# mj129/Tramba

Measured on AMD Instinct MI355X. Metric: images/sec fwd Tramba-V 384x384, higher is better.
Workload: dtype bf16; 1 GPU; Tramba-V (VMamba-B encoder) 384x384 bf16 inference, batch 4 per GPU, random-init weights (seed 1026), randn images; global_batch=4, launch=hipGraph replay, decoder guide branches on a side stream

## Files before the change

### tramba_amd/csrc/linear.hip

```cpp
#include <stdlib.h>
#include <string.h>

#include <type_traits>

#include "common.h"

namespace tramba {

typedef __attribute__((ext_vector_type(8))) short frag8_t;
typedef __attribute__((ext_vector_type(8))) _Float16 frag8h_t;
typedef __attribute__((ext_vector_type(16))) float acc16_t;

template <typename T> struct Mfma;
template <> struct Mfma<__hip_bfloat16> {
    static constexpr int KSTEP = 16;
    using frag = frag8_t;
    static __device__ __forceinline__ acc16_t run(frag a, frag b, acc16_t c)
    {
        typedef __attribute__((ext_vector_type(8))) __bf16 bf8;
        return __builtin_amdgcn_mfma_f32_32x32x16_bf16(__builtin_bit_cast(bf8, a), __builtin_bit_cast(bf8, b), c, 0, 0, 0);
    }
};
template <> struct Mfma<__half> {
    static constexpr int KSTEP = 16;
// ... 694 lines not shown
    TRAMBA_DSR128_(a[3], aa[3], S); TRAMBA_DSR128_(b[3], ba[3], S)
        if constexpr ((STG & 3) == 0) { TRAMBA_RD_STG_(0, 4096); }
        else if constexpr ((STG & 3) == 1) { TRAMBA_RD_STG_(16384, 20480); }
        else if constexpr ((STG & 3) == 2) { TRAMBA_RD_STG_(32768, 36864); }
        else { TRAMBA_RD_STG_(49152, 53248); }
#undef TRAMBA_RD_STG_
        if constexpr (LNIN) {
            asm volatile("s_waitcnt lgkmcnt(8)" : "+v"(sv[0]), "+v"(sv[1]) : : "memory");
#pragma unroll
            for (int i = 0; i < 2; ++i)
#pragma unroll
                for (int e = 0; e < 4; ++e) {
                    rs1[i] = dot2_ones<T>(sv[i][e], rs1[i]);
                    rs2[i] = dot2_self<T>(sv[i][e], rs2[i]);
                }
        }
        asm volatile("s_waitcnt lgkmcnt(6)" : "+v"(a[0]), "+v"(b[0]) : : "memory");
        acc[0][0] = Mfma<T>::run(b[0], a[0], acc[0][0]);
        asm volatile("s_waitcnt lgkmcnt(4)" : "+v"(a[1]), "+v"(b[1]) : : "memory");
        acc[0][0] = Mfma<T>::run(b[1], a[1], acc[0][0]);
        asm volatile("s_waitcnt lgkmcnt(2)" : "+v"(a[2]), "+v"(b[2]) : : "memory");
        acc[0][0] = Mfma<T>::run(b[2], a[2], acc[0][0]);
        asm volatile("s_waitcnt lgkmcnt(0)" : "+v"(a[3]), "+v"(b[3]) : : "memory");
        acc[0][0] = Mfma<T>::run(b[3], a[3], acc[0][0]);
    };
    int kt0 = 0;
    for (; kt0 + NSTG <= nk; kt0 += NSTG) {
        kstep(kt0, std::integral_constant<int, 0>{});
        kstep(kt0 + 1, std::integral_constant<int, 1>{});
        if constexpr (NSTG > 2) kstep(kt0 + 2, std::integral_constant<int, 2>{});
        if constexpr (NSTG > 3) kstep(kt0 + 3, std::integral_constant<int, 3>{});
        if constexpr (NSTG > 4) {
            kstep(kt0 + 4, std::integral_constant<int, 4>{});
            kstep(kt0 + 5, std::integral_constant<int, 5>{});
            kstep(kt0 + 6, std::integral_constant<int, 6>{});
            kstep(kt0 + 7, std::integral_constant<int, 7>{});
        }
    }
    if (kt0 < nk) kstep(kt0, std::integral_constant<int, 0>{});
    if constexpr (NSTG > 2) {
        if (kt0 + 1 < nk) kstep(kt0 + 1, std::integral_constant<int, 1>{});
    }
    if constexpr (NSTG > 3) {
        if (kt0 + 2 < nk) kstep(kt0 + 2, std::integral_constant<int, 2>{});
    }
    if constexpr (NSTG > 4) {
        if (kt0 + 3 < nk) kstep(kt0 + 3, std::integral_constant<int, 3>{});
        if (kt0 + 4 < nk) kstep(kt0 + 4, std::integral_constant<int, 4>{});
        if (kt0 + 5 < nk) kstep(kt0 + 5, std::integral_constant<int, 5>{});
        if (kt0 + 6 < nk) kstep(kt0 + 6, std::integral_constant<int, 6>{});
    }
    __syncthreads();
    if constexpr (LNIN) {
        float2 *rowstat = reinterpret_cast<float2 *>(lds + LDS_BYTES);
#pragma unroll
        for (int i = 0; i < 2; ++i) {
            float s1 = rs1[i], s2 = rs2[i];
#pragma unroll
            for (int m = 1; m < 8; m <<= 1) {
                s1 += __shfl_xor(s1, m, 64);
                s2 += __shfl_xor(s2, m, 64);
            }
            const float mean = s1 / (float)K;
            const float var = fmaxf(s2 / (float)K - mean * mean, 0.f);
            if ((tid & 7) == 0) rowstat[(tid >> 3) + 32 * i] = make_float2(mean, rsqrtf(var + li.eps));
        }
        tile_epilogue<T, TO, BM, BN>(acc, lds, bias, res, y, M, N, act, m0, n0, li.colsum,
                                     reinterpret_cast<const float2 *>(lds + LDS_BYTES));
    } else {
        tile_epilogue<T, TO, BM, BN>(acc, lds, bias, res, y, M, N, act, m0, n0, nullptr, nullptr, DUAL ? y_pre : nullptr);
    }
#endif
}

enum { A_PLAIN = 0, A_TWO = 1, A_CONV = 2 };
struct ASrc {
    const void *x2;
    int k1;
    ConvGeom cg;
    unsigned abytes;
};

#define TRAMBA_DSR128_(OUT, ADDR, OFF) asm volatile("ds_read_b128 %0, %1 offset:" #OFF : "=v"(OUT) : "v"(ADDR) : "memory")
template <typename T, typename TO, int NSTG, bool LNIN = false, bool DUAL = false, int ASRC = A_PLAIN>
__global__ __launch_bounds__(512, ASRC == A_CONV && NSTG == 3 ? 6 : 1) void linear_pc_kernel(const T *__restrict__ x, const T *__restrict__ w,
                                                       const float *__restrict__ bias, const T *__restrict__ res,
                                                       TO *__restrict__ y, long M, int N, int K, int act,
                                                       LnIn li = LnIn{nullptr, 0.f}, TO *__restrict__ y_pre = nullptr,
                                                       ASrc as = ASrc{nullptr, 0, ConvGeom{0, 0, 0, 0, 0}, 0u})
{
#if defined(__HIP_DEVICE_COMPILE__)
    constexpr int BM = 64, BN = 64;
    constexpr int TILE_BYTES = (BM + BN) * kBK * 2;
    constexpr int EPI_BYTES = BM * (BN + 4) * 4;
    constexpr int LDS_BYTES = NSTG * TILE_BYTES > EPI_BYTES ? NSTG * TILE_BYTES : EPI_BYTES;
    static_assert(NSTG == 3 || NSTG == 4, "stage index = kt % NSTG with the loop unrolled by NSTG");
    __shared__ __attribute__((aligned(1024))) unsigned char lds[LDS_BYTES + (LNIN ? BM * 8 : 0)];
    typedef __attribute__((address_space(3))) void lds_void;

    const int tid = threadIdx.x, lane = tid & 63;
    const int wave = __builtin_amdgcn_readfirstlane(tid >> 6);
    const bool loader = wave >= 4;
    const int cw = wave & 3;
    const int wm = cw >> 1, wn = cw & 1;
    const int r32 = lane & 31, hi = lane >> 5;
    long m0;
    int n0;
    {
        const unsigned nblk = gridDim.x * gridDim.y, lin = blockIdx.y * gridDim.x + blockIdx.x;
        const unsigned q = nblk >> 3, r = nblk & 7, xcd = lin & 7, slot = lin >> 3;
        const unsigned t = xcd * q + (xcd < r ? xcd : r) + slot;
        m0 = (long)(t / gridDim.x) * BM;
        n0 = (int)(t % gridDim.x) * BN;
    }
    const int nk = K / kBK;
    const unsigned rowb = (unsigned)K * 2u;
    const long mrows = M - m0 < BM ? M - m0 : BM;
    const int nrows = N - n0 < BN ? N - n0 : BN;
    const bool stage_b = cw >= 2;
    __amdgpu_buffer_rsrc_t rs, rsx;
    unsigned voff[4];
    unsigned lx[4] = {0u, 0u, 0u, 0u}, ly[4] = {0u, 0u, 0u, 0u};
    unsigned(&voff2)[4] = lx;
    unsigned(&chy)[4] = lx, (&cwx)[4] = ly;
    int nsw = nk;
    unsigned hlim = 0xffffffffu, wlim = 0xffffffffu;
    int ccs = 0, cdy = 0, cdx = 0;
    if constexpr (ASRC == A_TWO) {
        const int ka = as.k1;
        const unsigned rowa = (unsigned)ka * 2u, rowa2 = (unsigned)(K - ka) * 2u;
        rs = stage_b ? make_rsrc(w + (long)n0 * K, (unsigned)nrows * rowb) : make_rsrc(x + m0 * ka, (unsigned)mrows * rowa);
        rsx = stage_b ? rs : make_rsrc((const T *)as.x2 + m0 * (K - ka), (unsigned)mrows * rowa2);
        if (!stage_b) nsw = ka / kBK;
#pragma unroll
        for (int j = 0; j < 4; ++j) {
            const int row = ((cw & 1) * 4 + j) * 8 + (lane >> 3);
            const int c = (lane & 7) ^ ((row >> 1) & 7);
            voff[j] = (unsigned)row * (stage_b ? rowb : rowa) + (unsigned)c * 16u;
            voff2[j] = (unsigned)row * (stage_b ? rowb : rowa2) + (unsigned)c * 16u;
        }
    } else if constexpr (ASRC == A_CONV) {
        rs = stage_b ? make_rsrc(w + (long)n0 * K, (unsigned)nrows * rowb) : make_rsrc(x, as.abytes);
        if (!stage_b) {
            hlim = (unsigned)as.cg.hin;
            wlim = (unsigned)as.cg.win;
        }
#pragma unroll
        for (int j = 0; j < 4; ++j) {
            const int row = ((cw & 1) * 4 + j) * 8 + (lane >> 3);
            const int c = (lane & 7) ^ ((row >> 1) & 7);
            if (stage_b) {
                voff[j] = (unsigned)row * rowb + (unsigned)c * 16u;
                chy[j] = cwx[j] = 0u;
            } else {
                const long gr = m0 + row;
                const bool ok = gr < M;
                const unsigned pix = ok ? (unsigned)gr : 0u;
                const unsigned wo = pix % (unsigned)as.cg.wout, t = pix / (unsigned)as.cg.wout;
                const unsigned ho = t % (unsigned)as.cg.hout, b = t / (unsigned)as.cg.hout;
                chy[j] = (unsigned)(ok ? 2 * (int)ho - 1 : -4);
                cwx[j] = (unsigned)(2 * (int)wo - 1);
                voff[j] = ((b * (unsigned)as.cg.hin + chy[j]) * (unsigned)as.cg.win + cwx[j]) * ((unsigned)as.cg.cin * 2u) +
                          (unsigned)c * 16u;
            }
        }
    } else {
        rs = stage_b ? make_rsrc(w + (long)n0 * K, (unsigned)nrows * rowb) : make_rsrc(x + m0 * K, (unsigned)mrows * rowb);
#pragma unroll
        for (int j = 0; j < 4; ++j) {
            const int row = ((cw & 1) * 4 + j) * 8 + (lane >> 3);
            const int c = (lane & 7) ^ ((row >> 1) & 7);
            voff[j] = (unsigned)row * rowb + (unsigned)c * 16u;
        }
    }
    unsigned char *mine = lds + (stage_b ? BM * kBK * 2 : 0) + (cw & 1) * 4096;
    auto issue = [&](int kt, int stg) {
        if constexpr (ASRC == A_TWO) {
            const bool first = kt < nsw;
            const __amdgpu_buffer_rsrc_t rsel = first ? rs : rsx;
            const unsigned so = (unsigned)(first ? kt : kt - nsw) * (kBK * 2);
#pragma unroll
            for (int j = 0; j < 4; ++j)
                __builtin_amdgcn_raw_ptr_buffer_load_lds(rsel, (lds_void *)(mine + stg * TILE_BYTES + j * 1024), 16,
                                                         first ? voff[j] : voff2[j], so, 0, 0);
        } else if constexpr (ASRC == A_CONV) {
            const unsigned so = stage_b ? (unsigned)kt * (kBK * 2)
                                        : (unsigned)((cdy * as.cg.win + cdx) * as.cg.cin + ccs * kBK) * 2u;
#pragma unroll
            for (int j = 0; j < 4; ++j) {
                const unsigned hy = chy[j] + (unsigned)cdy, wx = cwx[j] + (unsigned)cdx;
                unsigned out = (hy < hlim && wx < wlim) ? 0u : 1u;
                asm volatile("" : "+v"(out));
                __builtin_amdgcn_raw_ptr_buffer_load_lds(rs, (lds_void *)(mine + stg * TILE_BYTES + j * 1024), 16,
                                                         (voff[j] + so) | (out << 31), 0, 0, 0);
            }
            if (++ccs == as.cg.cin / kBK) {
                ccs = 0;
                if (++cdx == 3) { cdx = 0; ++cdy; }
            }
        } else {
            const unsigned so = (unsigned)kt * (kBK * 2);
#pragma unroll
            for (int j = 0; j < 4; ++j)
                __builtin_amdgcn_raw_ptr_buffer_load_lds(rs, (lds_void *)(mine + stg * TILE_BYTES + j * 1024), 16, voff[j], so,
                                                         0, 0);
        }
    };
    const unsigned lbase = (unsigned)(size_t)(__attribute__((address_space(3))) unsigned char *)lds;
    unsigned(&aad)[4] = lx, (&bad)[4] = ly;
    if (ASRC == A_PLAIN || !loader) {
        const int ra_ = wm * 32 + r32, rb_ = wn * 32 + r32;
        const unsigned a0 = lbase + (unsigned)(ra_ * 128 + ((hi ^ ((ra_ >> 1) & 7)) * 16));
        const unsigned b0 = lbase + (unsigned)(BM * kBK * 2 + rb_ * 128 + ((hi ^ ((rb_ >> 1) & 7)) * 16));
#pragma unroll
        for (int kk = 0; kk < 4; ++kk) {
            aad[kk] = a0 ^ (unsigned)(kk * 32);
            bad[kk] = b0 ^ (unsigned)(kk * 32);
        }
    }
    acc16_t acc[1][1];
#pragma unroll
    for (int r = 0; r < 16; ++r) acc[0][0][r] = 0.f;
    const int lt = tid & 255;
    float rs1[2] = {0.f, 0.f}, rs2[2] = {0.f, 0.f};
    const unsigned sad = lbase + (unsigned)((lt >> 3) * 128 + (lt & 7) * 16);

    constexpr int DEPTH = NSTG - 1;
    if (loader) {
#pragma unroll
        for (int t = 0; t < DEPTH; ++t)
            if (t < nk) issue(t, t);
    }
    auto kstep = [&](int kt, auto stg_c) {
        constexpr int STG = decltype(stg_c)::value;
        if (loader) {
            const int later = nk - 1 - kt;
            if (later >= DEPTH - 1) {
                if constexpr (DEPTH == 2) asm volatile("s_waitcnt vmcnt(4)" ::: "memory");
                else asm volatile("s_waitcnt vmcnt(8)" ::: "memory");
            } else {
                switch (later) {
                case 0: asm volatile("s_waitcnt vmcnt(0)" ::: "memory"); break;
                default: asm volatile("s_waitcnt vmcnt(4)" ::: "memory"); break;
                }
            }
        }
        __builtin_amdgcn_s_barrier();
        asm volatile("" ::: "memory");
        if (loader) {
            if (kt + DEPTH < nk) issue(kt + DEPTH, (STG + DEPTH) % NSTG);
        } else {
            frag8_t a[4], b[4];
            v4u_t sv[2];
            if constexpr (LNIN) {
                if constexpr (STG == 0) { TRAMBA_DSR128_(sv[0], sad, 0); TRAMBA_DSR128_(sv[1], sad, 4096); }
                else if constexpr (STG == 1) { TRAMBA_DSR128_(sv[0], sad, 16384); TRAMBA_DSR128_(sv[1], sad, 20480); }
                else if constexpr (STG == 2) { TRAMBA_DSR128_(sv[0], sad, 32768); TRAMBA_DSR128_(sv[1], sad, 36864); }
                else { TRAMBA_DSR128_(sv[0], sad, 49152); TRAMBA_DSR128_(sv[1], sad, 53248); }
            }
#define TRAMBA_RD_STG_(S)                                                                            \
    TRAMBA_DSR128_(a[0], aad[0], S); TRAMBA_DSR128_(b[0], bad[0], S); TRAMBA_DSR128_(a[1], aad[1], S); \
    TRAMBA_DSR128_(b[1], bad[1], S); TRAMBA_DSR128_(a[2], aad[2], S); TRAMBA_DSR128_(b[2], bad[2], S); \
    TRAMBA_DSR128_(a[3], aad[3], S); TRAMBA_DSR128_(b[3], bad[3], S)
            if constexpr (STG == 0) { TRAMBA_RD_STG_(0); }
            else if constexpr (STG == 1) { TRAMBA_RD_STG_(16384); }
            else if constexpr (STG == 2) { TRAMBA_RD_STG_(32768); }
            else { TRAMBA_RD_STG_(49152); }
#undef TRAMBA_RD_STG_
            if constexpr (LNIN) {
                asm volatile("s_waitcnt lgkmcnt(8)" : "+v"(sv[0]), "+v"(sv[1]) : : "memory");
#pragma unroll
                for (int i = 0; i < 2; ++i)
#pragma unroll
                    for (int e = 0; e < 4; ++e) {
                        rs1[i] = dot2_ones<T>(sv[i][e], rs1[i]);
                        rs2[i] = dot2_self<T>(sv[i][e], rs2[i]);
                    }
            }
            asm volatile("s_waitcnt lgkmcnt(6)" : "+v"(a[0]), "+v"(b[0]) : : "memory");
            acc[0][0] = Mfma<T>::run(b[0], a[0], acc[0][0]);
            __builtin_amdgcn_sched_barrier(0);
            asm volatile("s_waitcnt lgkmcnt(4)" : "+v"(a[1]), "+v"(b[1]) : : "memory");
            acc[0][0] = Mfma<T>::run(b[1], a[1], acc[0][0]);
            __builtin_amdgcn_sched_barrier(0);
            asm volatile("s_waitcnt lgkmcnt(2)" : "+v"(a[2]), "+v"(b[2]) : : "memory");
            acc[0][0] = Mfma<T>::run(b[2], a[2], acc[0][0]);
            __builtin_amdgcn_sched_barrier(0);
            asm volatile("s_waitcnt lgkmcnt(0)" : "+v"(a[3]), "+v"(b[3]) : : "memory");
            acc[0][0] = Mfma<T>::run(b[3], a[3], acc[0][0]);
        }
    };
    int kt0 = 0;
    for (; kt0 + NSTG <= nk; kt0 += NSTG) {
        kstep(kt0, std::integral_constant<int, 0>{});
        kstep(kt0 + 1, std::integral_constant<int, 1>{});
        kstep(kt0 + 2, std::integral_constant<int, 2>{});
        if constexpr (NSTG > 3) kstep(kt0 + 3, std::integral_constant<int, 3>{});
    }
    if (kt0 < nk) kstep(kt0, std::integral_constant<int, 0>{});
    if (kt0 + 1 < nk) kstep(kt0 + 1, std::integral_constant<int, 1>{});
    if constexpr (NSTG > 3) {
        if (kt0 + 2 < nk) kstep(kt0 + 2, std::integral_constant<int, 2>{});
    }
    __syncthreads();
    if constexpr (LNIN) {
        float2 *rowstat = reinterpret_cast<float2 *>(lds + LDS_BYTES);
        if (!loader) {
#pragma unroll
            for (int i = 0; i < 2; ++i) {
                float s1 = rs1[i], s2 = rs2[i];
#pragma unroll
                for (int m = 1; m < 8; m <<= 1) {
                    s1 += __shfl_xor(s1, m, 64);
                    s2 += __shfl_xor(s2, m, 64);
                }
                const float mean = s1 / (float)K;
                const float var = fmaxf(s2 / (float)K - mean * mean, 0.f);
                if ((lt & 7) == 0) rowstat[(lt >> 3) + 32 * i] = make_float2(mean, rsqrtf(var + li.eps));
            }
        }
        tile_epilogue<T, TO, BM, BN, 512>(acc, lds, bias, res, y, M, N, act, m0, n0, li.colsum,
                                          reinterpret_cast<const float2 *>(lds + LDS_BYTES));
    } else {
        tile_epilogue<T, TO, BM, BN, 512>(acc, lds, bias, res, y, M, N, act, m0, n0, nullptr, nullptr, DUAL ? y_pre : nullptr);
    }
#endif
}
#undef TRAMBA_DSR128_

template <typename T> __device__ __forceinline__ unsigned pack2_(float a, float b);
template <> __device__ __forceinline__ unsigned pack2_<__hip_bfloat16>(float a, float b)
{
    unsigned pk = 0u;
#if defined(__HIP_DEVICE_COMPILE__)
    asm("v_cvt_pk_bf16_f32 %0, %1, %2" : "=v"(pk) : "v"(a), "v"(b));
#endif
    return pk;
}
template <> __device__ __forceinline__ unsigned pack2_<__half>(float a, float b)
{
    unsigned pk = 0u;
#if defined(__HIP_DEVICE_COMPILE__)
    asm("v_cvt_pk_f16_f32 %0, %1, %2" : "=v"(pk) : "v"(a), "v"(b));
#endif
    return pk;
}
template <typename T> __device__ __forceinline__ float unpack_lo_(unsigned v);
template <typename T> __device__ __forceinline__ float unpack_hi_(unsigned v);
template <> __device__ __forceinline__ float unpack_lo_<__hip_bfloat16>(unsigned v) { return __builtin_bit_cast(float, v << 16); }
template <> __device__ __forceinline__ float unpack_hi_<__hip_bfloat16>(unsigned v) { return __builtin_bit_cast(float, v & 0xffff0000u); }
template <> __device__ __forceinline__ float unpack_lo_<__half>(unsigned v) { return (float)__builtin_bit_cast(_Float16, (unsigned short)(v & 0xffffu)); }
template <> __device__ __forceinline__ float unpack_hi_<__half>(unsigned v) { return (float)__builtin_bit_cast(_Float16, (unsigned short)(v >> 16)); }

typedef unsigned v2u_t __attribute__((ext_vector_type(2)));

#define TRAMBA_DSR128I_(OUT, ADDR, OFF) asm volatile("ds_read_b128 %0, %1 offset:%2" : "=v"(OUT) : "v"(ADDR), "i"(OFF) : "memory")
#define TRAMBA_VMCNT_(N) asm volatile("s_waitcnt vmcnt(%0)" ::"n"(N) : "memory")

template <typename T, int K, int NCW, bool LNIN, bool DUAL, bool RES>
__global__ __launch_bounds__(256, 2) void linear_ws_kernel(const T *__restrict__ x, const T *__restrict__ w,
                                                          const float *__restrict__ bias, const T *__restrict__ res,
                                                          T *__restrict__ y, long M, int N, int act, LnIn li,
                                                          T *__restrict__ y_pre, int npanel, int gt)
{
#if defined(__HIP_DEVICE_COMPILE__)
    static_assert(K == 128 || K == 256, "row = one or two 256-byte bank rows");
    static_assert(NCW * K <= 512, "the wave's B fragments stay in <= 128 registers");
    static_assert((((K == 128 && NCW <= 2) ? 6 : 4) - 1) * 32 * K * 2 + 512 <= 65535, "the last ring stage inside ds_read's 16-bit offset");
    static_assert((((K == 128 && NCW <= 2) ? 6 : 4) - 1) * (NCW * 2 * (DUAL ? 2 : 1)) +
                          (((K == 128 && NCW <= 2) ? 6 : 4) - 2) * ((RES ? NCW * 4 : 0) + K / 64) <= 63,
                  "the counted vmcnt fits its 6-bit field");
    static_assert(!(DUAL && RES), "a dual-output launch has no residual");
    static_assert(!RES || NCW <= 2, "residual rows are prefetched into registers");
    constexpr int KB = K / 16;
    constexpr int RB = K * 2;
    constexpr int TILE_BYTES = 32 * RB;
    constexpr int NSTG = (K == 128 && NCW <= 2) ? 6 : 4;
    constexpr int PPW = K / 64;
    constexpr int PANEL = 128 * NCW;
    constexpr int S = NCW * 2 * (DUAL ? 2 : 1);
    constexpr int RL = RES ? NCW * 4 : 0;
    __shared__ __attribute__((aligned(1024))) unsigned char lds[NSTG * TILE_BYTES + PANEL * 8];
    typedef __attribute__((address_space(3))) void lds_void;
    float *lbias = reinterpret_cast<float *>(lds + NSTG * TILE_BYTES);
    float *lcs = lbias + PANEL;

    const int tid = threadIdx.x, lane = tid & 63;
    const int wv = __builtin_amdgcn_readfirstlane(tid >> 6);
    const int r32 = lane & 31, hi = lane >> 5;
    const int pn = blockIdx.x % npanel, g0 = blockIdx.x / npanel;
    const int n0 = pn * PANEL, n0w = n0 + wv * (NCW * 32);
    const long T32 = (M + 31) / 32;
    const int nt = g0 < T32 ? (int)((T32 - g0 + gt - 1) / gt) : 0;

    frag8_t bf[NCW][KB];
#pragma unroll
    for (int cb = 0; cb < NCW; ++cb)
#pragma unroll
        for (int kb = 0; kb < KB; ++kb)
            bf[cb][kb] = *reinterpret_cast<const frag8_t *>(w + (long)(n0w + cb * 32 + r32) * K + kb * 16 + hi * 8);
    for (int i = tid; i < PANEL; i += 256) {
        lbias[i] = bias ? bias[n0 + i] : 0.f;
        lcs[i] = LNIN ? li.colsum[n0 + i] : 0.f;
    }
    __syncthreads();

    const __amdgpu_buffer_rsrc_t rsx = make_rsrc(x, (unsigned)(M * RB));
    unsigned voff[PPW];
#pragma unroll
    for (int j = 0; j < PPW; ++j) {
        const int lo = (wv * PPW + j) * 1024 + lane * 16;
// ... 129 lines not shown
                v4f_t cf4 = {0.f, 0.f, 0.f, 0.f};
                if constexpr (LNIN) cf4 = __builtin_bit_cast(v4f_t, cq[g]);
#pragma unroll
                for (int q = 0; q < 4; ++q) {
                    float v = acc[cb][4 * g + q];
                    if constexpr (LNIN) v = rstd * fmaf(-mean, cf4[q], v);
                    o[4 * g + q] = v + bf4[q];
                }
            }
            if constexpr (DUAL) {
#pragma unroll
                for (int g = 0; g < 4; ++g) {
                    pp[g][0] = pack2_<T>(o[4 * g], o[4 * g + 1]);
                    pp[g][1] = pack2_<T>(o[4 * g + 2], o[4 * g + 3]);
                }
            }
            if (act == TRAMBA_ACT_GELU) {
#pragma unroll
                for (int e = 0; e < 16; ++e) o[e] = geluf_(o[e]);
            } else if (act == TRAMBA_ACT_SILU) {
#pragma unroll
                for (int e = 0; e < 16; ++e) o[e] = siluf_(o[e]);
            }
#pragma unroll
            for (int g = 0; g < 4; ++g) {
                if constexpr (RES) {
                    const v2u_t r2 = rv[cb * 4 + g];
                    o[4 * g + 0] += unpack_lo_<T>(r2[0]);
                    o[4 * g + 1] += unpack_hi_<T>(r2[0]);
                    o[4 * g + 2] += unpack_lo_<T>(r2[1]);
                    o[4 * g + 3] += unpack_hi_<T>(r2[1]);
                }
                pk[g][0] = pack2_<T>(o[4 * g], o[4 * g + 1]);
                pk[g][1] = pack2_<T>(o[4 * g + 2], o[4 * g + 3]);
            }
#pragma unroll
            for (int pr = 0; pr < 2; ++pr) {
                const auto w0 = __builtin_amdgcn_permlane32_swap(pk[2 * pr][0], pk[2 * pr + 1][0], false, false);
                const auto w1 = __builtin_amdgcn_permlane32_swap(pk[2 * pr][1], pk[2 * pr + 1][1], false, false);
                const unsigned a0 = w0[0], b0 = w0[1], a1 = w1[0], b1 = w1[1];
                const v4u_t out = {a0, a1, b0, b1};
                __builtin_amdgcn_raw_buffer_store_b128(out, rsy, yoff + (unsigned)((cb * 32 + pr * 16) * 2), so_y, 0);
                if constexpr (DUAL) {
                    const auto u0 = __builtin_amdgcn_permlane32_swap(pp[2 * pr][0], pp[2 * pr + 1][0], false, false);
                    const auto u1 = __builtin_amdgcn_permlane32_swap(pp[2 * pr][1], pp[2 * pr + 1][1], false, false);
                    const unsigned c0 = u0[0], d0 = u0[1], c1 = u1[0], d1 = u1[1];
                    const v4u_t outp = {c0, c1, d0, d1};
                    __builtin_amdgcn_raw_buffer_store_b128(outp, rsp, yoff + (unsigned)((cb * 32 + pr * 16) * 2), so_y, 0);
                }
            }
        }
    };
    for (int t0 = 0; t0 < nt; t0 += NSTG) {
        tile_step(t0, std::integral_constant<int, 0>{});
        if (t0 + 1 < nt) tile_step(t0 + 1, std::integral_constant<int, 1>{});
        if (t0 + 2 < nt) tile_step(t0 + 2, std::integral_constant<int, 2>{});
        if (t0 + 3 < nt) tile_step(t0 + 3, std::integral_constant<int, 3>{});
        if constexpr (NSTG > 4) {
            if (t0 + 4 < nt) tile_step(t0 + 4, std::integral_constant<int, 4>{});
            if (t0 + 5 < nt) tile_step(t0 + 5, std::integral_constant<int, 5>{});
        }
    }
    asm volatile("s_waitcnt vmcnt(0)" ::: "memory");
#endif
}
#undef TRAMBA_DSR128I_
#undef TRAMBA_VMCNT_

static bool ws_rule(long m, int n, int k, int kind )
{
    if (k != 128 || n < 256) return false;
    return kind == 1 ? m >= 16384 : m >= 65536;
}

static int pc_rule(long tiles64, int k, int kind)
{
    if (kind == 1) return tiles64 <= 320 ? 3 : 0;
    if (kind == 2) return (k <= 256 && tiles64 >= 4096) ? 0 : 3;
    if (k >= 2048 && tiles64 <= 256) return 4;
    if (k >= 2048 && tiles64 <= 320) return 0;
    return 3;
}

static int ws_ncw(long m, int n, int k)
{
    if (k != 128 && k != 256) return 0;
    if ((double)m * n * 2.0 >= 2147483648.0 || (double)(m + 32) * k * 2.0 >= 2147483648.0) return 0;
    int ncw = 256 / k;
    while (ncw >= 1 && n % (128 * ncw)) ncw >>= 1;
    return ncw;
}

template <typename T, int K, bool LNIN, bool DUAL, bool RES>
static void launch_ws(int ncw, const void *x, const void *w, const float *bias, const void *res, void *y, long m, int n, int act,
                      LnIn li, void *y_pre, hipStream_t s)
{
    const int npanel = n / (128 * ncw);
    const long t32 = (m + 31) / 32;
    const long resident = 256L * (K == 128 ? 3 : 2);
    long gt = resident / npanel;
    if (gt > t32) gt = t32;
    if (gt < 1) gt = 1;
    dim3 grid((unsigned)(gt * npanel)), block(256);
#define WS_(NCW_)                                                                                                      \
    hipLaunchKernelGGL((linear_ws_kernel<T, K, NCW_, LNIN, DUAL, RES>), grid, block, 0, s, (const T *)x, (const T *)w, bias, \
                       (const T *)res, (T *)y, m, n, act, li, (T *)y_pre, npanel, (int)gt)
    if constexpr (K == 128) {
        if (ncw == 2) { WS_(2); } else { WS_(1); }
    } else {
        WS_(1);
    }
#undef WS_
}

template <typename T, bool LNIN, bool DUAL>
static void launch_ws_k(int ncw, const void *x, const void *w, const float *bias, const void *res, void *y, long m, int n, int k,
                        int act, LnIn li, void *y_pre, hipStream_t s)
{
    if (k == 128) {
        if (res) { if constexpr (!DUAL) launch_ws<T, 128, LNIN, false, true>(ncw, x, w, bias, res, y, m, n, act, li, y_pre, s); }
        else launch_ws<T, 128, LNIN, DUAL, false>(ncw, x, w, bias, res, y, m, n, act, li, y_pre, s);
    } else {
        if (res) { if constexpr (!DUAL) launch_ws<T, 256, LNIN, false, true>(ncw, x, w, bias, res, y, m, n, act, li, y_pre, s); }
        else launch_ws<T, 256, LNIN, DUAL, false>(ncw, x, w, bias, res, y, m, n, act, li, y_pre, s);
    }
}

constexpr int DMA_SHORT_K = 256;

enum GemmKind { GEMM_PLAIN = 0, GEMM_LN = 1, GEMM_DUAL = 2, GEMM_TWO_SRC, GEMM_CONV };
enum class GemmForm {
    WS,
    PC3, PC4,
    DMA2, DMA3, DMA4,
    LEAN,
    TILED128, TILED64, TILED64_PF3
};
struct GemmPlan {
    GemmForm form;
    int ncw;
};

static GemmPlan gemm_plan(GemmKind kind, long m, int n, int k, int act, bool same_dtype, bool a_dma = true)
{
    int tune = tramba_tune_get(TRAMBA_TUNE_GEMM_TILE);
    if ((kind == GEMM_TWO_SRC || kind == GEMM_CONV) && a_dma && tune != 18 && k % 64 == 0 &&
        (double)k * 2.0 * 128.0 < 2147483648.0) {
        const long tiles64 = ((m + 63) / 64) * ((n + 63) / 64);
        return {pc_rule(tiles64, k, GEMM_PLAIN) == 4 ? GemmForm::PC4 : GemmForm::PC3, 0};
    }
    if (kind == GEMM_TWO_SRC) return {GemmForm::LEAN, 0};
    if (kind == GEMM_CONV || k % 64 != 0 || (double)k * 2.0 * 128.0 >= 2147483648.0) {
        const long big = ((m + 127) / 128) * ((n + 127) / 128);
        if (big >= 2048 && k >= 1024) return {GemmForm::TILED128, 0};
        return {k <= 128 ? GemmForm::TILED64 : GemmForm::TILED64_PF3, 0};
    }
    if (tune == 7 && kind != GEMM_PLAIN) tune = 0;
    if (tune == 0 || tune == 19) {
        const bool ws_act = act == TRAMBA_ACT_NONE || act == TRAMBA_ACT_GELU || act == TRAMBA_ACT_SILU;
        const int ncw = same_dtype && ws_act ? ws_ncw(m, n, k) : 0;
        if (ncw && (tune == 19 ? m >= 64 : ws_rule(m, n, k, kind))) return {GemmForm::WS, ncw};
    }
    switch (tune) {
    case 7: return {GemmForm::DMA4, 0};
    case 13: return {GemmForm::DMA2, 0};
    case 14: return {GemmForm::DMA3, 0};
    case 16: return {GemmForm::PC3, 0};
    case 17: return {GemmForm::PC4, 0};
    }
    const long tiles64 = ((m + 63) / 64) * ((n + 63) / 64);
    const int pc = tune == 18 ? 0 : pc_rule(tiles64, k, kind);
    if (pc) return {pc == 4 ? GemmForm::PC4 : GemmForm::PC3, 0};
    if (k <= DMA_SHORT_K && tiles64 >= 1024) return {GemmForm::DMA2, 0};
    if (kind == GEMM_PLAIN && tiles64 <= 256 && k >= 1024) return {GemmForm::DMA4, 0};
    return {GemmForm::DMA3, 0};
}

struct GemmArgs {
    const void *x, *w;
    const float *bias;
    const void *res;
    void *y;
    long m;
    int n, k, act;
    LnIn li{nullptr, 0.f};
    void *y_pre = nullptr;
    const void *x2 = nullptr;
    int k1 = 0;
    ConvGeom cg{0, 0, 0, 0, 0};
    unsigned abytes = 0;
};

template <typename T, typename TO, bool LNIN = false, bool DUAL = false, bool CONV = false>
static void launch_gemm(const GemmPlan &p, const GemmArgs &a, hipStream_t s)
{
    const T *x = (const T *)a.x, *w = (const T *)a.w, *res = (const T *)a.res;
    TO *y = (TO *)a.y, *y_pre = (TO *)a.y_pre;
    const long m = a.m;
    const int n = a.n, k = a.k, act = a.act;
    const dim3 g64((n + 63) / 64, (unsigned)((m + 63) / 64)), g128((n + 127) / 128, (unsigned)((m + 127) / 128));
    switch (p.form) {
    case GemmForm::WS:
        launch_ws_k<T, LNIN, DUAL>(p.ncw, a.x, a.w, a.bias, a.res, a.y, m, n, k, act, a.li, a.y_pre, s);
        break;
    case GemmForm::PC3:
    case GemmForm::PC4: {
        const bool four = p.form == GemmForm::PC4;
        if constexpr (CONV) {
            const ASrc as{nullptr, 0, a.cg, a.abytes};
            if (four) hipLaunchKernelGGL((linear_pc_kernel<T, TO, 4, false, false, A_CONV>), g64, dim3(512), 0, s, x, w, a.bias, res, y, m, n, k, act, a.li, y_pre, as);
            else hipLaunchKernelGGL((linear_pc_kernel<T, TO, 3, false, false, A_CONV>), g64, dim3(512), 0, s, x, w, a.bias, res, y, m, n, k, act, a.li, y_pre, as);
            break;
        }
        if constexpr (!LNIN && !DUAL) {
            if (a.x2) {
                const ASrc as{a.x2, a.k1, a.cg, 0u};
                if (four) hipLaunchKernelGGL((linear_pc_kernel<T, TO, 4, false, false, A_TWO>), g64, dim3(512), 0, s, x, w, a.bias, res, y, m, n, k, act, a.li, y_pre, as);
                else hipLaunchKernelGGL((linear_pc_kernel<T, TO, 3, false, false, A_TWO>), g64, dim3(512), 0, s, x, w, a.bias, res, y, m, n, k, act, a.li, y_pre, as);
                break;
            }
        }
        if (four) hipLaunchKernelGGL((linear_pc_kernel<T, TO, 4, LNIN, DUAL>), g64, dim3(512), 0, s, x, w, a.bias, res, y, m, n, k, act, a.li, y_pre);
        else hipLaunchKernelGGL((linear_pc_kernel<T, TO, 3, LNIN, DUAL>), g64, dim3(512), 0, s, x, w, a.bias, res, y, m, n, k, act, a.li, y_pre);
        break;
    }
    case GemmForm::DMA2:
        hipLaunchKernelGGL((linear_dma_kernel<T, TO, 2, LNIN, DUAL>), g64, dim3(256), 0, s, x, w, a.bias, res, y, m, n, k, act, a.li, y_pre);
        break;
    case GemmForm::DMA3:
        hipLaunchKernelGGL((linear_dma_kernel<T, TO, 3, LNIN, DUAL>), g64, dim3(256), 0, s, x, w, a.bias, res, y, m, n, k, act, a.li, y_pre);
        break;
    case GemmForm::DMA4:
        if constexpr (!LNIN && !DUAL)
            hipLaunchKernelGGL((linear_dma_kernel<T, TO, 4>), g64, dim3(256), 0, s, x, w, a.bias, res, y, m, n, k, act, a.li, y_pre);
        break;
    case GemmForm::LEAN:
        hipLaunchKernelGGL((linear_lean_kernel<T, TO, 64, 64, 1>), g64, dim3(256), 0, s, x, w, a.bias, res, y, m, n, k, act,
                           (const T *)a.x2, a.k1);
        break;
    case GemmForm::TILED128:
        hipLaunchKernelGGL((linear_tiled_kernel<T, TO, 128, 128, 2, CONV>), g128, dim3(256), 0, s, x, w, a.bias, res, y, m, n, k, act, a.cg);
        break;
    case GemmForm::TILED64:
        hipLaunchKernelGGL((linear_tiled_kernel<T, TO, 64, 64, 1, CONV>), g64, dim3(256), 0, s, x, w, a.bias, res, y, m, n, k, act, a.cg);
        break;
    case GemmForm::TILED64_PF3:
        hipLaunchKernelGGL((linear_tiled_kernel<T, TO, 64, 64, 3, CONV>), g64, dim3(256), 0, s, x, w, a.bias, res, y, m, n, k, act, a.cg);
        break;
    }
}

template <bool LNIN = false>
static void launch_gemm16(const GemmPlan &p, const GemmArgs &a, int dtype, int out_dtype, hipStream_t s)
{
    if (dtype == TRAMBA_BF16) {
        if (out_dtype == TRAMBA_F32) launch_gemm<__hip_bfloat16, float, LNIN>(p, a, s);
        else launch_gemm<__hip_bfloat16, __hip_bfloat16, LNIN>(p, a, s);
    } else {
        if (out_dtype == TRAMBA_F32) launch_gemm<__half, float, LNIN>(p, a, s);
        else launch_gemm<__half, __half, LNIN>(p, a, s);
    }
}

template <typename TO>
__global__ __launch_bounds__(256) void linear32_kernel(const float *__restrict__ x, const float *__restrict__ w,
                                                      const float *__restrict__ bias, const float *__restrict__ res,
                                                      TO *__restrict__ y, long M, int N, int K, int act)
{
    const int lane = threadIdx.x & 63, wave = threadIdx.x >> 6;
    const long m0 = (long)blockIdx.y * 128 + (wave >> 1) * 64;
    const int n0 = blockIdx.x * 128 + (wave & 1) * 64;
    if (m0 >= M || n0 >= N) return;
    acc16_t acc[2][2];
#pragma unroll
    for (int i = 0; i < 2; ++i)
#pragma unroll
        for (int j = 0; j < 2; ++j)
#pragma unroll
            for (int r = 0; r < 16; ++r) acc[i][j][r] = 0.f;
    const int r32 = lane & 31, kh = lane >> 5;
    for (int k0 = 0; k0 < K; k0 += 2) {
        const int k = k0 + kh;
        float a[2], b[2];
#pragma unroll
        for (int i = 0; i < 2; ++i) {
            const long row = m0 + i * 32 + r32;
            a[i] = (row < M && k < K) ? x[row * K + k] : 0.f;
        }
#pragma unroll
        for (int j = 0; j < 2; ++j) {
            const int col = n0 + j * 32 + r32;
            b[j] = (col < N && k < K) ? w[(long)col * K + k] : 0.f;
        }
#pragma unroll
        for (int i = 0; i < 2; ++i)
#pragma unroll
            for (int j = 0; j < 2; ++j)
                acc[i][j] = __builtin_amdgcn_mfma_f32_32x32x2f32(a[i], b[j], acc[i][j], 0, 0, 0);
    }
#pragma unroll
    for (int i = 0; i < 2; ++i)
#pragma unroll
        for (int j = 0; j < 2; ++j)
            store_tile<float, TO>(acc[i][j], y, bias, res, m0 + i * 32, n0 + j * 32, M, N, act, lane);
}

}

// ... 169 lines not shown
```

### tramba_amd/csrc/runtime.hip

```cpp
#include <stdarg.h>
#include <string.h>

#include <algorithm>
#include <mutex>
#include <vector>

#include "common.h"

namespace tramba {

static thread_local char g_err[512] = "";

void set_error(const char *fmt, ...)
{
    va_list ap;
    va_start(ap, fmt);
    vsnprintf(g_err, sizeof(g_err), fmt, ap);
    va_end(ap);
}

struct ProfState {
    bool enabled = false;
    double min_units = 0.0;
    std::vector<std::pair<hipEvent_t, hipEvent_t>> events;
// ... 1 lines not shown
};
static ProfState g_prof[TRAMBA_PROF_COUNT];
static std::mutex g_prof_mu;

ProfScope::ProfScope(int w, hipStream_t s, double units) : which(w), stream(s), on(false), start(nullptr)
{
    if (w < 0 || w >= TRAMBA_PROF_COUNT || !g_prof[w].enabled || units < g_prof[w].min_units) return;
    hipStreamCaptureStatus st = hipStreamCaptureStatusNone;
    if (hipStreamIsCapturing(s, &st) != hipSuccess || st != hipStreamCaptureStatusNone) return;
    if (hipEventCreate(&start) != hipSuccess) return;
    on = true;
    g_prof[w].units += units;
    (void)hipEventRecord(start, s);
}

ProfScope::~ProfScope()
{
    if (!on) return;
    hipEvent_t stop;
    if (hipEventCreate(&stop) != hipSuccess) return;
    (void)hipEventRecord(stop, stream);
    std::lock_guard<std::mutex> lk(g_prof_mu);
    g_prof[which].events.emplace_back(start, stop);
}

unsigned *g_deverr_host = nullptr;
static unsigned *g_deverr_dev = nullptr;
static std::once_flag g_deverr_once;

static void deverr_alloc()
{
    unsigned *h = nullptr, *d = nullptr;
    if (hipHostMalloc((void **)&h, 64, hipHostMallocMapped | hipHostMallocPortable | hipHostMallocCoherent) != hipSuccess) {
        (void)hipGetLastError();
        return;
    }
    *h = 0u;
    if (hipHostGetDevicePointer((void **)&d, h, 0) != hipSuccess) {
        (void)hipGetLastError();
        (void)hipHostFree(h);
        return;
    }
    g_deverr_dev = d;
    set_mailbox_err_word(d);
    g_deverr_host = h;
}

MailboxCtl mailbox_ctl(hipStream_t s)
{
    if (!g_deverr_host) {
        hipStreamCaptureStatus st = hipStreamCaptureStatusNone;
        if (hipStreamIsCapturing(s, &st) == hipSuccess && st == hipStreamCaptureStatusNone) std::call_once(g_deverr_once, deverr_alloc);
    }
    const int t = tramba_tune_get(TRAMBA_TUNE_MAILBOX_SKIP);
    return MailboxCtl{t > 0 ? t : -1};
}

int dev_error_report(const char *file, int line)
{
    const unsigned code = __atomic_exchange_n(g_deverr_host, 0u, __ATOMIC_RELAXED);
    if (!code) return TRAMBA_OK;
    set_error("device error word 0x%x%s (seen at %s:%d): a kernel launched EARLIER by this library failed on the device and its "
              "output holds NaN", code, (code & TRAMBA_DEVERR_MAILBOX) ? " [fused scan: carry mailbox timed out]" : "", file, line);
    return TRAMBA_ERR_HIP;
}

}

using namespace tramba;

extern "C" const char *tramba_last_error(void) { return g_err; }
extern "C" int tramba_device_error(void)
{
    if (g_deverr_host && *(volatile unsigned *)g_deverr_host) return dev_error_report("tramba_device_error", 0);
    return TRAMBA_OK;
}
extern "C" int tramba_abi_version(void) { return 7; }

static int g_tune[TRAMBA_TUNE_COUNT] = {0};
extern "C" int tramba_tune_set(int knob, int value)
{
    TRAMBA_CHECK(knob >= 0 && knob < TRAMBA_TUNE_COUNT, "tune knob %d out of range", knob);
    TRAMBA_CHECK(knob != 5, "tune knob 5 (the weight-gradient form) is retired");
    TRAMBA_CHECK(knob != TRAMBA_TUNE_GEMM_TILE || value == 0 || value == 7 || value == 13 || value == 14 || (value >= 16 && value <= 19),
                 "TRAMBA_TUNE_GEMM_TILE %d is retired or unknown (kept: 0, 7, 13, 14, 16-19)", value);
    g_tune[knob] = value;
    return TRAMBA_OK;
}
extern "C" int tramba_tune_get(int knob) { return knob >= 0 && knob < TRAMBA_TUNE_COUNT ? g_tune[knob] : 0; }

extern "C" int tramba_profile_enable(int which, int enable)
{
    TRAMBA_CHECK(which >= 0 && which < TRAMBA_PROF_COUNT, "profile class %d out of range", which);
    std::lock_guard<std::mutex> lk(g_prof_mu);
    g_prof[which].enabled = enable != 0;
    return TRAMBA_OK;
}

extern "C" int tramba_profile_min_units(int which, double min_units)
{
    TRAMBA_CHECK(which >= 0 && which < TRAMBA_PROF_COUNT, "profile class %d out of range", which);
    std::lock_guard<std::mutex> lk(g_prof_mu);
    g_prof[which].min_units = min_units;
    return TRAMBA_OK;
}

extern "C" int tramba_profile_read(int which, double *total_ms, double *total_units)
{
    TRAMBA_CHECK(which >= 0 && which < TRAMBA_PROF_COUNT, "profile class %d out of range", which);
    std::lock_guard<std::mutex> lk(g_prof_mu);
    ProfState &p = g_prof[which];
    double ms = 0.0;
    int n = 0;
    for (auto &ev : p.events) {
        (void)hipEventSynchronize(ev.second);
        float t = 0.f;
        if (hipEventElapsedTime(&t, ev.first, ev.second) == hipSuccess) {
            ms += t;
            ++n;
        }
        (void)hipEventDestroy(ev.first);
        (void)hipEventDestroy(ev.second);
    }
    p.events.clear();
    if (total_ms) *total_ms = ms;
    if (total_units) *total_units = p.units;
    p.units = 0.0;
    return n;
}


extern "C" int tramba_scan_family_k(int family)
{
    switch (family) {
    case TRAMBA_SCAN_RASTER:
    case TRAMBA_SCAN_LINE:
    case TRAMBA_SCAN_WINDOW:
    case TRAMBA_SCAN_DILATION: return 4;
    case TRAMBA_SCAN_HELIX: return 8;
    default: set_error("unknown scan family %d", family); return TRAMBA_ERR_ARG;
    }
}

extern "C" int tramba_default_window(int h)
{
    switch (h) {
    case 12: return 4;
    case 24: return 8;
    case 48: return 12;
    case 96: return 16;
    default: break;
    }
    if (h >= 64 && h % 16 == 0) return 16;
    for (int ws = 8; ws >= 2; ws /= 2)
        if (h % ws == 0 && h > ws) return ws;
    return 1;
}

static void raster_rows(int h, int w, int32_t *out)
{
    const int L = h * w;
    for (int i = 0; i < L; ++i) {
        out[i] = i;
        out[L + i] = (i % h) * w + (i / h);
    }
    for (int i = 0; i < L; ++i) {
        out[2 * L + i] = out[L - 1 - i];
        out[3 * L + i] = out[2 * L - 1 - i];
// ... 120 lines not shown
```

Measured before the change: 854.9 img/s.

## Add 128-row tile variant of producer-consumer GEMM for mid-sized K=1024 shapes

Adds a BM=128 instantiation of the warp-specialized linear kernel. Loader waves fill both A (128 rows) and B tiles into three LDS stages, and each compute wave runs two MFMAs per k-slice that share one B fragment. It is picked by default for K=1024 GEMMs with a moderate tile count and wide N, aiming to halve B-operand traffic and raise MFMA density per LDS read. The cost is fewer blocks and more LDS per block (occupancy hint of 4), which may underfill the GPU on smaller grids.

```diff
diff --git a/tramba_amd/csrc/linear.hip b/tramba_amd/csrc/linear.hip
--- a/tramba_amd/csrc/linear.hip
+++ b/tramba_amd/csrc/linear.hip
@@ -800,19 +800,21 @@
 };
 
 #define TRAMBA_DSR128_(OUT, ADDR, OFF) asm volatile("ds_read_b128 %0, %1 offset:" #OFF : "=v"(OUT) : "v"(ADDR) : "memory")
-template <typename T, typename TO, int NSTG, bool LNIN = false, bool DUAL = false, int ASRC = A_PLAIN>
-__global__ __launch_bounds__(512, ASRC == A_CONV && NSTG == 3 ? 6 : 1) void linear_pc_kernel(const T *__restrict__ x, const T *__restrict__ w,
+#define TRAMBA_DSR128C_(OUT, ADDR, OFF) asm volatile("ds_read_b128 %0, %1 offset:%2" : "=v"(OUT) : "v"(ADDR), "i"(OFF) : "memory")
+template <typename T, typename TO, int NSTG, bool LNIN = false, bool DUAL = false, int ASRC = A_PLAIN, int BM = 64>
+__global__ __launch_bounds__(512, BM == 128 ? 4 : ASRC == A_CONV && NSTG == 3 ? 6 : 1) void linear_pc_kernel(const T *__restrict__ x, const T *__restrict__ w,
                                                        const float *__restrict__ bias, const T *__restrict__ res,
                                                        TO *__restrict__ y, long M, int N, int K, int act,
                                                        LnIn li = LnIn{nullptr, 0.f}, TO *__restrict__ y_pre = nullptr,
                                                        ASrc as = ASrc{nullptr, 0, ConvGeom{0, 0, 0, 0, 0}, 0u})
 {
 #if defined(__HIP_DEVICE_COMPILE__)
-    constexpr int BM = 64, BN = 64;
+    constexpr int BN = 64;
     constexpr int TILE_BYTES = (BM + BN) * kBK * 2;
     constexpr int EPI_BYTES = BM * (BN + 4) * 4;
     constexpr int LDS_BYTES = NSTG * TILE_BYTES > EPI_BYTES ? NSTG * TILE_BYTES : EPI_BYTES;
     static_assert(NSTG == 3 || NSTG == 4, "stage index = kt % NSTG with the loop unrolled by NSTG");
+    static_assert(BM == 64 || (BM == 128 && NSTG == 3 && ASRC == A_PLAIN), "the 128-row tile: 3 stages (2 x 72 KB on a CU), plain A operand");
     __shared__ __attribute__((aligned(1024))) unsigned char lds[LDS_BYTES + (LNIN ? BM * 8 : 0)];
     typedef __attribute__((address_space(3))) void lds_void;
 
@@ -844,7 +846,24 @@
     int nsw = nk;
     unsigned hlim = 0xffffffffu, wlim = 0xffffffffu;
     int ccs = 0, cdy = 0, cdx = 0;
-    if constexpr (ASRC == A_TWO) {
+    if constexpr (BM == 128) {
+        rs = make_rsrc(x + m0 * K, (unsigned)mrows * rowb);
+        rsx = make_rsrc(w + (long)n0 * K, (unsigned)nrows * rowb);
+        if (loader) {
+#pragma unroll
+            for (int j = 0; j < 4; ++j) {
+                const int row = (cw * 4 + j) * 8 + (lane >> 3);
+                const int c = (lane & 7) ^ ((row >> 1) & 7);
+                lx[j] = (unsigned)row * rowb + (unsigned)c * 16u;
+            }
+#pragma unroll
+            for (int j = 0; j < 2; ++j) {
+                const int row = (cw * 2 + j) * 8 + (lane >> 3);
+                const int c = (lane & 7) ^ ((row >> 1) & 7);
+                ly[j] = (unsigned)row * rowb + (unsigned)c * 16u;
+            }
+        }
+    } else if constexpr (ASRC == A_TWO) {
         const int ka = as.k1;
         const unsigned rowa = (unsigned)ka * 2u, rowa2 = (unsigned)(K - ka) * 2u;
         rs = stage_b ? make_rsrc(w + (long)n0 * K, (unsigned)nrows * rowb) : make_rsrc(x + m0 * ka, (unsigned)mrows * rowa);
@@ -893,7 +912,17 @@
     }
     unsigned char *mine = lds + (stage_b ? BM * kBK * 2 : 0) + (cw & 1) * 4096;
     auto issue = [&](int kt, int stg) {
-        if constexpr (ASRC == A_TWO) {
+        if constexpr (BM == 128) {
+            const unsigned so = (unsigned)kt * (kBK * 2);
+            unsigned char *st = lds + stg * TILE_BYTES;
+#pragma unroll
+            for (int j = 0; j < 4; ++j)
+                __builtin_amdgcn_raw_ptr_buffer_load_lds(rs, (lds_void *)(st + cw * 4096 + j * 1024), 16, lx[j], so, 0, 0);
+#pragma unroll
+            for (int j = 0; j < 2; ++j)
+                __builtin_amdgcn_raw_ptr_buffer_load_lds(rsx, (lds_void *)(st + BM * kBK * 2 + cw * 2048 + j * 1024), 16, ly[j], so,
+                                                         0, 0);
+        } else if constexpr (ASRC == A_TWO) {
             const bool first = kt < nsw;
             const __amdgpu_buffer_rsrc_t rsel = first ? rs : rsx;
             const unsigned so = (unsigned)(first ? kt : kt - nsw) * (kBK * 2);
@@ -926,8 +955,8 @@
     };
     const unsigned lbase = (unsigned)(size_t)(__attribute__((address_space(3))) unsigned char *)lds;
     unsigned(&aad)[4] = lx, (&bad)[4] = ly;
-    if (ASRC == A_PLAIN || !loader) {
-        const int ra_ = wm * 32 + r32, rb_ = wn * 32 + r32;
+    if (BM == 128 ? !loader : (ASRC == A_PLAIN || !loader)) {
+        const int ra_ = wm * (BM / 2) + r32, rb_ = wn * 32 + r32;
         const unsigned a0 = lbase + (unsigned)(ra_ * 128 + ((hi ^ ((ra_ >> 1) & 7)) * 16));
         const unsigned b0 = lbase + (unsigned)(BM * kBK * 2 + rb_ * 128 + ((hi ^ ((rb_ >> 1) & 7)) * 16));
 #pragma unroll
@@ -936,11 +965,16 @@
             bad[kk] = b0 ^ (unsigned)(kk * 32);
         }
     }
-    acc16_t acc[1][1];
-#pragma unroll
-    for (int r = 0; r < 16; ++r) acc[0][0][r] = 0.f;
+    acc16_t acc[BM / 64][1];
+#pragma unroll
+    for (int i = 0; i < BM / 64; ++i)
+#pragma unroll
+        for (int r = 0; r < 16; ++r) acc[i][0][r] = 0.f;
     const int lt = tid & 255;
-    float rs1[2] = {0.f, 0.f}, rs2[2] = {0.f, 0.f};
+    constexpr int NRS = BM / 32;
+    float rs1[NRS], rs2[NRS];
+#pragma unroll
+    for (int i = 0; i < NRS; ++i) rs1[i] = rs2[i] = 0.f;
     const unsigned sad = lbase + (unsigned)((lt >> 3) * 128 + (lt & 7) * 16);
 
     constexpr int DEPTH = NSTG - 1;
@@ -949,6 +983,49 @@
         for (int t = 0; t < DEPTH; ++t)
             if (t < nk) issue(t, t);
     }
+    auto lstep128 = [&](int kt, int stg) {
+        if (kt + 1 < nk) asm volatile("s_waitcnt vmcnt(6)" ::: "memory");
+        else asm volatile("s_waitcnt vmcnt(0)" ::: "memory");
+        __builtin_amdgcn_s_barrier();
+        asm volatile("" ::: "memory");
+        if (kt + DEPTH < nk) issue(kt + DEPTH, stg);
+    };
+    auto mstep128 = [&](auto stg_c) {
+        constexpr int STG = decltype(stg_c)::value;
+        __builtin_amdgcn_s_barrier();
+        asm volatile("" ::: "memory");
+        if constexpr (BM == 128) {
+            frag8_t a[3][2], b[3];
+            v4u_t sv[2];
+            constexpr int S = STG * TILE_BYTES, SVR = LNIN ? 2 : 0;
+#define TRAMBA_RD_KK_(KK, SL) \
+    TRAMBA_DSR128C_(a[SL][0], aad[KK], S); TRAMBA_DSR128C_(a[SL][1], aad[KK], S + 4096); TRAMBA_DSR128C_(b[SL], bad[KK], S)
+#define TRAMBA_MM_KK_(SL, LEFT)                                                                                        \
+    asm volatile("s_waitcnt lgkmcnt(%3)" : "+v"(a[SL][0]), "+v"(a[SL][1]), "+v"(b[SL]) : "n"(LEFT) : "memory");       \
+    acc[0][0] = Mfma<T>::run(b[SL], a[SL][0], acc[0][0]);                                                             \
+    acc[1][0] = Mfma<T>::run(b[SL], a[SL][1], acc[1][0]);                                                             \
+    __builtin_amdgcn_sched_barrier(0)
+#define TRAMBA_STAT_(I0, LEFT)                                                                                        \
+    asm volatile("s_waitcnt lgkmcnt(%2)" : "+v"(sv[0]), "+v"(sv[1]) : "n"(LEFT) : "memory");                          \
+    _Pragma("unroll") for (int i = 0; i < 2; ++i) _Pragma("unroll") for (int e = 0; e < 4; ++e) {                     \
+        rs1[I0 + i] = dot2_ones<T>(sv[i][e], rs1[I0 + i]);                                                            \
+        rs2[I0 + i] = dot2_self<T>(sv[i][e], rs2[I0 + i]);                                                            \
+    }
+            if constexpr (LNIN) { TRAMBA_DSR128C_(sv[0], sad, S); TRAMBA_DSR128C_(sv[1], sad, S + 4096); }
+            TRAMBA_RD_KK_(0, 0); TRAMBA_RD_KK_(1, 1); TRAMBA_RD_KK_(2, 2);
+            if constexpr (LNIN) { TRAMBA_STAT_(0, 9); }
+            TRAMBA_MM_KK_(0, 6);
+            if constexpr (LNIN) { TRAMBA_DSR128C_(sv[0], sad, S + 8192); TRAMBA_DSR128C_(sv[1], sad, S + 12288); }
+            TRAMBA_RD_KK_(3, 0);
+            TRAMBA_MM_KK_(1, 6 + SVR);
+            TRAMBA_MM_KK_(2, 3 + SVR);
+            if constexpr (LNIN) { TRAMBA_STAT_(2, 3); }
+            TRAMBA_MM_KK_(0, 0);
+#undef TRAMBA_RD_KK_
+#undef TRAMBA_MM_KK_
+#undef TRAMBA_STAT_
+        }
+    };
     auto kstep = [&](int kt, auto stg_c) {
         constexpr int STG = decltype(stg_c)::value;
         if (loader) {
@@ -1009,6 +1086,23 @@
         }
     };
     int kt0 = 0;
+    if constexpr (BM == 128) {
+        if (loader) {
+            int stg = DEPTH;
+            for (; kt0 < nk; ++kt0) {
+                lstep128(kt0, stg);
+                stg = stg == NSTG - 1 ? 0 : stg + 1;
+            }
+        } else {
+            for (; kt0 + NSTG <= nk; kt0 += NSTG) {
+                mstep128(std::integral_constant<int, 0>{});
+                mstep128(std::integral_constant<int, 1>{});
+                mstep128(std::integral_constant<int, 2>{});
+            }
+            if (kt0 < nk) mstep128(std::integral_constant<int, 0>{});
+            if (kt0 + 1 < nk) mstep128(std::integral_constant<int, 1>{});
+        }
+    } else {
     for (; kt0 + NSTG <= nk; kt0 += NSTG) {
         kstep(kt0, std::integral_constant<int, 0>{});
         kstep(kt0 + 1, std::integral_constant<int, 1>{});
@@ -1020,12 +1114,13 @@
     if constexpr (NSTG > 3) {
         if (kt0 + 2 < nk) kstep(kt0 + 2, std::integral_constant<int, 2>{});
     }
+    }
     __syncthreads();
     if constexpr (LNIN) {
         float2 *rowstat = reinterpret_cast<float2 *>(lds + LDS_BYTES);
         if (!loader) {
 #pragma unroll
-            for (int i = 0; i < 2; ++i) {
+            for (int i = 0; i < NRS; ++i) {
                 float s1 = rs1[i], s2 = rs2[i];
 #pragma unroll
                 for (int m = 1; m < 8; m <<= 1) {
@@ -1045,6 +1140,7 @@
 #endif
 }
 #undef TRAMBA_DSR128_
+#undef TRAMBA_DSR128C_
 
 template <typename T> __device__ __forceinline__ unsigned pack2_(float a, float b);
 template <> __device__ __forceinline__ unsigned pack2_<__hip_bfloat16>(float a, float b)
@@ -1340,6 +1436,14 @@
     return 3;
 }
 
+static bool m128_rule(long m, int n, int k, int kind)
+{
+    if (k != 1024 || m > 2304) return false;
+    const long tiles64 = ((m + 63) / 64) * ((n + 63) / 64);
+    if (tiles64 < 288 || tiles64 > 1152) return false;
+    return kind == 1 ? n >= 4096 : n >= 512;
+}
+
 static int ws_ncw(long m, int n, int k)
 {
     if (k != 128 && k != 256) return 0;
@@ -1390,6 +1494,7 @@
 enum class GemmForm {
     WS,
     PC3, PC4,
+    PC3_M128,
     DMA2, DMA3, DMA4,
     LEAN,
     TILED128, TILED64, TILED64_PF3
@@ -1414,6 +1519,8 @@
         return {k <= 128 ? GemmForm::TILED64 : GemmForm::TILED64_PF3, 0};
     }
     if (tune == 7 && kind != GEMM_PLAIN) tune = 0;
+    const bool no_m128 = tune == 22;
+    if (no_m128) tune = 0;
     if (tune == 0 || tune == 19) {
         const bool ws_act = act == TRAMBA_ACT_NONE || act == TRAMBA_ACT_GELU || act == TRAMBA_ACT_SILU;
         const int ncw = same_dtype && ws_act ? ws_ncw(m, n, k) : 0;
@@ -1425,7 +1532,9 @@
     case 14: return {GemmForm::DMA3, 0};
     case 16: return {GemmForm::PC3, 0};
     case 17: return {GemmForm::PC4, 0};
-    }
+    case 21: return {GemmForm::PC3_M128, 0};
+    }
+    if (tune == 0 && !no_m128 && m128_rule(m, n, k, kind)) return {GemmForm::PC3_M128, 0};
     const long tiles64 = ((m + 63) / 64) * ((n + 63) / 64);
     const int pc = tune == 18 ? 0 : pc_rule(tiles64, k, kind);
     if (pc) return {pc == 4 ? GemmForm::PC4 : GemmForm::PC3, 0};
@@ -1482,6 +1591,11 @@
         else hipLaunchKernelGGL((linear_pc_kernel<T, TO, 3, LNIN, DUAL>), g64, dim3(512), 0, s, x, w, a.bias, res, y, m, n, k, act, a.li, y_pre);
         break;
     }
+    case GemmForm::PC3_M128:
+        if constexpr (!CONV)
+            hipLaunchKernelGGL((linear_pc_kernel<T, TO, 3, LNIN, DUAL, A_PLAIN, 128>), dim3((n + 63) / 64, (unsigned)((m + 127) / 128)),
+                               dim3(512), 0, s, x, w, a.bias, res, y, m, n, k, act, a.li, y_pre);
+        break;
     case GemmForm::DMA2:
         hipLaunchKernelGGL((linear_dma_kernel<T, TO, 2, LNIN, DUAL>), g64, dim3(256), 0, s, x, w, a.bias, res, y, m, n, k, act, a.li, y_pre);
         break;
diff --git a/tramba_amd/csrc/runtime.hip b/tramba_amd/csrc/runtime.hip
--- a/tramba_amd/csrc/runtime.hip
+++ b/tramba_amd/csrc/runtime.hip
@@ -107,8 +107,8 @@
 {
     TRAMBA_CHECK(knob >= 0 && knob < TRAMBA_TUNE_COUNT, "tune knob %d out of range", knob);
     TRAMBA_CHECK(knob != 5, "tune knob 5 (the weight-gradient form) is retired");
-    TRAMBA_CHECK(knob != TRAMBA_TUNE_GEMM_TILE || value == 0 || value == 7 || value == 13 || value == 14 || (value >= 16 && value <= 19),
-                 "TRAMBA_TUNE_GEMM_TILE %d is retired or unknown (kept: 0, 7, 13, 14, 16-19)", value);
+    TRAMBA_CHECK(knob != TRAMBA_TUNE_GEMM_TILE || value == 0 || value == 7 || value == 13 || value == 14 || (value >= 16 && value <= 19) || value == 21 || value == 22,
+                 "TRAMBA_TUNE_GEMM_TILE %d is retired or unknown (kept: 0, 7, 13, 14, 16-19, 21, 22)", value);
     g_tune[knob] = value;
     return TRAMBA_OK;
 }
```

New measurement: 849.9 img/s. No clear change (-0.6%).
